# lucadellalib/audiocodecs

Measured on AMD Instinct MI355X. Metric: encode+decode audio-sec/s, EnCodec-24k 8cb, higher is better.
Workload: dtype f32 (GEMM-shaped kernels and LSTM products: operands as two scaled fp16 planes, 3 partial products, fp32 accumulate -- split16.h)

## Files before the change

audiocodecs_amd/csrc/ac_api.hip:

```cpp
#include "core.h"
#include "tap_route.h"

extern "C" {

int ac_version(void) { return 400; }

int ac_create(const ac_config* cfg, ac_handle** out) {
    if (!cfg || !out) return AC_EINVAL;
    *out = nullptr;
    if (cfg->struct_size != (int32_t)sizeof(ac_config)) return AC_EINVAL;
    if (cfg->num_ratios < 1 || cfg->num_ratios > AC_MAX_RATIOS || cfg->num_filters < 1 || cfg->hidden_size < 16 ||
        cfg->hidden_size % 16 || cfg->compress < 1 || cfg->num_lstm_layers < 1 || cfg->num_lstm_layers > 2 || cfg->codebook_size % 32 ||
        cfg->codebook_size < 16 || cfg->num_quantizers < 1 || cfg->kernel_size < 1 || cfg->kernel_size > 8 ||
        cfg->last_kernel_size < 1 || cfg->last_kernel_size > 8 || cfg->residual_kernel_size < 1 || cfg->residual_kernel_size > 8)
        return AC_EINVAL;
    int ndev = 0;
    if (hipGetDeviceCount(&ndev) != hipSuccess || ndev <= cfg->device || cfg->device < 0) return AC_ENODEV;
    ac_handle* h = new (std::nothrow) ac_handle();
    if (!h) return AC_ENOMEM;
    h->cfg = *cfg;
    h->hop = 1;
    for (int i = 0; i < cfg->num_ratios; ++i) h->hop *= cfg->upsampling_ratios[i];
    h->D = cfg->num_filters << cfg->num_ratios;
    *out = h;
// ... 16 lines not shown
    if (ends(".weight_g")) k = k.substr(0, k.size() - 9) + ".parametrizations.weight.original0";
    else if (ends(".weight_v")) k = k.substr(0, k.size() - 9) + ".parametrizations.weight.original1";
    return k;
}

int ac_load_weights(ac_handle* h, const char* name, const void* host_ptr, size_t bytes) {
    if (!h || !name || !host_ptr) return h ? fail(h, AC_EINVAL, "null argument") : AC_EINVAL;
    if (h->finalized) return fail(h, AC_ESTATE, "handle already finalized");
    if (bytes % 4) return fail(h, AC_EINVAL, "tensor '%s': byte size %zu is not a multiple of 4", name, bytes);
    const float* f = static_cast<const float*>(host_ptr);
    h->host[h->arch == ARCH_WAVTOK ? wavtok_key(name) : std::string(name)].assign(f, f + bytes / 4);
    return AC_OK;
}



static void latch_dev_switches(ac_handle* h) {
    auto num = [](const char* name, int dflt) { const char* v = std::getenv(name); return v && *v ? std::atoi(v) : dflt; };
    const char* e = std::getenv("AC_TAP_EPI");
    h->dev.tap_epi_staged = e && std::strcmp(e, "staged") == 0;
    h->dev.tap_dil = num("AC_TAP_DIL", 1);
    h->dev.tap_stagger = num("AC_TAP_STAGGER", 0);
    h->dev.tap_pick = num("AC_TAP_PICK", -1);
    h->dev.tap8 = num("AC_TAP8", -1);
    h->dev.tap8_form = num("AC_TAP8_FORM", 0);
    h->dev.tap8_spread = num("AC_TAP8_SPREAD", 1);
#ifdef AC_DEVELOPER
    h->dev.rb6_dbg = num("AC_RB6_DBG", 0);
    h->dev.lstm_dbg = num("AC_LSTM_DBG", 0);
#endif
    h->dev.rb_stream = num("AC_RB_STREAM", 1);
    h->dev.chain_stream = num("AC_CHAIN_STREAM", 1);
    h->dev.rb128_stream = num("AC_RB128_STREAM", 1);
    h->dev.front_seg = std::max(0, num("AC_FRONT_SEG", 0));
    h->dev.tail_seg = std::max(0, num("AC_TAIL_SEG", 0));
    h->dev.front_ldspad = std::max(0, num("AC_FRONT_LDSPAD", 0));
    h->dev.lstm_fuse_in = num("AC_LSTM_FUSE_IN", 1);
    const char* r = std::getenv("AC_RVQ");
    h->dev.rvq_exact = r && std::strcmp(r, "fp32") == 0;
    h->dev.prof_detail = num("AC_PROF_DETAIL", 0);
    h->dev.head_seq = num("AC_HEAD_SEQ", 0);
    h->dev.attn_exact = num("AC_ATTN_EXACT", 0);
    h->dev.dac_unit = num("AC_DAC_UNIT", 1);
    h->dev.mimi_tail = num("AC_MIMI_TAIL", 1);
    h->dev.mstream_skinny = num("AC_MSTREAM_SKINNY", -1);
}

int ac_debug_set(ac_handle* h, const char* key, int value) {
    if (!h || !key) return AC_EINVAL;
    struct { const char* k; int* v; } tab[] = {
        {"tap_epi_staged", &h->dev.tap_epi_staged}, {"tap_dil", &h->dev.tap_dil}, {"tap_stagger", &h->dev.tap_stagger}, {"tap_pick", &h->dev.tap_pick}, {"tap8", &h->dev.tap8}, {"tap8_form", &h->dev.tap8_form}, {"tap8_spread", &h->dev.tap8_spread},
        {"rb6_dbg", &h->dev.rb6_dbg}, {"rb_stream", &h->dev.rb_stream}, {"chain_stream", &h->dev.chain_stream}, {"rb128_stream", &h->dev.rb128_stream}, {"front_seg", &h->dev.front_seg}, {"tail_seg", &h->dev.tail_seg}, {"front_ldspad", &h->dev.front_ldspad},
        {"lstm_dbg", &h->dev.lstm_dbg}, {"lstm_fuse_in", &h->dev.lstm_fuse_in}, {"rvq_exact", &h->dev.rvq_exact}, {"prof_detail", &h->dev.prof_detail}, {"head_seq", &h->dev.head_seq}, {"attn_exact", &h->dev.attn_exact}, {"dac_unit", &h->dev.dac_unit}, {"mimi_tail", &h->dev.mimi_tail},
        {"mstream_skinny", &h->dev.mstream_skinny},
    };
#ifndef AC_DEVELOPER
    if (std::strcmp(key, "rb6_dbg") == 0 || std::strcmp(key, "lstm_dbg") == 0)
        return fail(h, AC_EINVAL, "ac_debug_set('%s'): a developer-build switch (timing modes with wrong results / fault injection); this is the product library", key);
#endif
    if (!h->finalized) return fail(h, AC_ESTATE, "ac_debug_set('%s'): the switches are latched by ac_finalize; set them afterwards", key);
    for (auto& t : tab)
        if (std::strcmp(t.k, key) == 0) {
            const bool nonneg = t.v == &h->dev.front_seg || t.v == &h->dev.tail_seg || t.v == &h->dev.front_ldspad || t.v == &h->dev.tap_stagger;
            if (nonneg && value < 0) return fail(h, AC_EINVAL, "ac_debug_set('%s', %d): the value must be >= 0", key, value);
            if (t.v == &h->dev.front_ldspad && value > 16384) return fail(h, AC_EINVAL, "ac_debug_set('front_ldspad', %d): at most 16384 bytes", value);
            if (t.v == &h->dev.tap8_form && (value < 0 || value > 5)) return fail(h, AC_EINVAL, "ac_debug_set('tap8_form', %d): 0 (cost model) .. 5", value);
            *t.v = value;
            return AC_OK;
        }
    return fail(h, AC_EINVAL, "ac_debug_set: unknown switch '%s'", key);
}

int ac_set_precision(ac_handle* h, int precision) {
    if (!h) return AC_EINVAL;
    if (h->finalized) return fail(h, AC_ESTATE, "ac_set_precision must precede ac_finalize (weights are packed for one arithmetic)");
    if (precision != AC_PRECISION_FP32 && precision != AC_PRECISION_FP32_EXACT) return fail(h, AC_EINVAL, "unknown precision %d", precision);
    h->precision = precision;
    return AC_OK;
}

int ac_finalize(ac_handle* h) {
    if (!h) return AC_EINVAL;
    if (h->finalized) return fail(h, AC_ESTATE, "handle already finalized");
    {
        int pr = h->precision;
// ... 587 lines not shown
```

audiocodecs_amd/csrc/core.h:

```cpp
#pragma once
#include <hip/hip_runtime.h>

#include <algorithm>
#include <cmath>
#include <cstdarg>
#include <cstdio>
#include <cstdlib>
#include <cstring>
#include <map>
#include <string>
#include <vector>

#include "../../include/audiocodecs_amd.h"
#include "lstm_consts.h"
#include "rvq_types.h"
#include "split16.h"
#include "tap_gemm.h"

using namespace ac;

namespace ac {
constexpr int THIN_MAXK = 8;
struct RbFused6Params;
}

namespace acimpl {


struct ConvSpec {
    std::string prefix;
    int transposed, cin, cout, k, s;
};

struct PackedGemm {
    size_t w_off = 0, b_off = 0;
    int N = 0, Ktot = 0;
    bool has_bias = true;
};

struct ResBlockPlan {
    int C;
    PackedGemm c3;
    PackedGemm fused;
    size_t w3f_off = 0, wff_off = 0;
    size_t winv3_off = 0, winvf_off = 0;
    size_t w3p_off = 0, wfp_off = 0;
    float hb0 = 0.f, hb1 = 0.f;
    bool has6 = false;
};

struct LstmPlan {
    int D, layers;
    std::vector<PackedGemm> ih;
    std::vector<size_t> hh_off;
    std::vector<size_t> ihpk_off;
    size_t persist_off = 0;
    size_t persist16_off = 0;
    size_t persist16_inv = 0;
    bool has_persist = false;
};

struct MimiTfLayer {
    PackedGemm qkv, o, fc1, fc2;
    size_t ln1_w = 0, ln1_b = 0, ln2_w = 0, ln2_b = 0, sc_a = 0, sc_m = 0;
};

struct MimiPlan {
    PackedGemm enc_stem, enc_final, down, dec_first, dec_head;
    std::vector<ResBlockPlan> enc_rb, dec_rb;
    std::vector<PackedGemm> enc_down, dec_up;
    std::vector<MimiTfLayer> enc_tf, dec_tf;
    size_t up_w = 0;
    PackedGemm in_proj;
    PackedGemm out_proj;
    size_t cb_plain = 0, cb_packed = 0, cb_ee = 0;
    size_t cb16 = 0, cb16_inv = 0;
    size_t rope_cos = 0, rope_sin = 0;
    int rope_T = 0;
    int D = 0;
    struct StreamM { size_t stem_f = 0, stem_inv = 0, head_f = 0, head_inv = 0; float sb0 = 0.f, sb1 = 0.f, fb0 = 0.f, fb1h = 0.f; bool stem_ok = false, head_ok = false; } sm;
};
// ... 58 lines not shown
    ac_mimi_config mcfg{};
    MimiPlan mimi;
    ac_dac_config dcfg{};
    DacPlan dac;
    ac_wavtok_config wcfg{};
    WavtokPlan wt;
    std::string err;
    std::map<std::string, std::vector<float>> host;
    bool finalized = false;
    float* blob = nullptr;
    size_t blob_floats = 0;
    int hop = 1, D = 0;
    PackedGemm enc_stem, enc_final;
    std::vector<ResBlockPlan> enc_rb;
    std::vector<PackedGemm> enc_down;
    LstmPlan enc_lstm, dec_lstm;
    PackedGemm dec_first, dec_head;
    std::vector<PackedGemm> dec_up;
    std::vector<ResBlockPlan> dec_rb;
    size_t cb_plain = 0, cb_packed = 0, cb_ee = 0;
    size_t cb16 = 0, cb16_inv = 0;
    struct ChainBounds { float sb0 = 0.f, sb1 = 0.f, fb0 = 0.f, fb1h = 0.f, fb1x = 0.f; bool ok = false; } enc_front, dec_tail;
    struct StreamImgs { size_t stem_f = 0, stem_inv = 0, down_f = 0, down_inv = 0, up_f = 0, up_inv = 0, head_f = 0, head_inv = 0; bool enc_ok = false, dec_ok = false; } simg;
    struct DevSwitches {
        int tap_epi_staged = 0;
        int tap_dil = 1;
        int tap_stagger = 0;
        int tap_pick = -1;
        int tap8 = -1;
        int tap8_form = 0;
        int tap8_spread = 1;
        int rb6_dbg = 0;
        int rb_stream = 1;
        int rb128_stream = 1;
        int chain_stream = 1;
        int front_seg = 0, tail_seg = 0;
        int front_ldspad = 0;
        int lstm_dbg = 0;
        int lstm_fuse_in = 1;
        int rvq_exact = 0;
        int prof_detail = 0;
        int attn_exact = 0;
        int dac_unit = 1;
        int mimi_tail = 1;
        int head_seq = 0;
        int mstream_skinny = -1;
    } dev;
    bool fuse_chains = true;
    float* dbg = nullptr;
    size_t dbg_cap = 0, dbg_used = 0;
    std::vector<const void*> lds_opted;
    std::map<size_t, size_t> w6_of;
    std::map<size_t, size_t> t6_of;
    std::map<size_t, size_t> t6inv_of;
    bool noncausal = false;
    bool has_enc = true, has_dec = true;
    bool gemm_fp32 = false;
    std::map<size_t, size_t> winv_of;
    std::map<const void*, int> mimi_streams;
    std::map<const void*, int> mimi_dstreams;
    struct EStreamReg {
        int B;
        std::vector<uint8_t> fresh;
    };
    std::map<const void*, EStreamReg> encodec_streams, encodec_dstreams;
    unsigned* amax_buf = nullptr;
// ... 207 lines not shown
        const int KS = H / 32;
        *img_off = reserve((size_t)Q * C * H);
        *inv_off = reserve((size_t)Q);
        std::vector<uint16_t> img((size_t)Q * C * H * 2);
        for (int q = 0; q < Q; ++q) {
            const float* e = &blob[plain + (size_t)q * C * H];
            const int se = row_scale(e, (size_t)C * H);
            blob[*inv_off + q] = s16_pow2(-se);
            for (int ct = 0; ct < C / 16; ++ct)
                for (int s = 0; s < KS; ++s)
                    for (int lane = 0; lane < 64; ++lane)
                        for (int e8 = 0; e8 < 8; ++e8) {
                            const int j = lane & 15, kq = lane >> 4;
                            const int dim = 16 * (2 * s + e8 / 4) + 4 * kq + e8 % 4;
                            uint16_t t[3];
                            split16h(e[(size_t)(ct * 16 + j) * H + dim], se, t);
                            const size_t base = ((((size_t)q * (C / 16) + ct) * KS + s) * 2) * 512 + (size_t)lane * 8 + e8;
                            img[base] = t[0];
                            img[base + 512] = t[1];
                        }
        }
        std::memcpy(&blob[*img_off], img.data(), img.size() * 2);
    }
    void pack_t6(const PackedGemm& g) {
        if (g.N != 64 || g.Ktot != 128 || !g.has_bias || h->t6_of.count(g.w_off)) return;
        std::vector<int> km(128);
        for (int k = 0; k < 128; ++k) km[k] = k;
        size_t ioff = 0;
        h->t6_of[g.w_off] = frag16(g.w_off, 64, 128, km, &ioff);
        if (use16()) h->t6inv_of[g.w_off] = ioff;
    }
    void rb6(ResBlockPlan& rb, bool sc) {
        const int C = rb.C, hid = C / 2;
        if ((C != 32 && C != 64 && C != 128) || rb.c3.N != hid || rb.c3.Ktot != 3 * C || rb.fused.N != C || rb.fused.Ktot != hid + (sc ? C : 0)) return;
        std::vector<int> k3(3 * C), kf;
        for (int k = 0; k < 3 * C; ++k) k3[k] = k;
        const int hcp = hid < 32 ? 32 : hid;
        for (int k = 0; k < hcp; ++k) kf.push_back(k < hid ? k : -1);
        for (int k = 0; sc && k < C; ++k) kf.push_back(hid + k);
        rb.w3f_off = frag16(rb.c3.w_off, hid, rb.c3.Ktot, k3, &rb.winv3_off);
        rb.wff_off = frag16(rb.fused.w_off, C, rb.fused.Ktot, kf, &rb.winvf_off);
        if ((C == 64 || C == 32 || C == 128) && use16()) {
            std::vector<int> k3p(k3.size()), kfp(kf.size());
            for (size_t k = 0; k < k3.size(); ++k) k3p[k] = k3[(k & ~(size_t)31) + ((k & 4) ? 16 : 0) + 4 * ((k >> 3) & 3) + (k & 3)];
            for (size_t k = 0; k < kf.size(); ++k) kfp[k] = kf[(k & ~(size_t)31) + ((k & 4) ? 16 : 0) + 4 * ((k >> 3) & 3) + (k & 3)];
            rb.w3p_off = frag16(rb.c3.w_off, hid, rb.c3.Ktot, k3p);
            rb.wfp_off = frag16(rb.fused.w_off, C, rb.fused.Ktot, kfp);
        }
        rb.hb0 = rb.hb1 = 0.f;
        for (int n = 0; n < hid; ++n) {
            double l1 = 0.0;
            for (int k = 0; k < rb.c3.Ktot; ++k) l1 += std::fabs((double)blob[rb.c3.w_off + (size_t)n * rb.c3.Ktot + k]);
            rb.hb1 = std::max(rb.hb1, (float)(l1 * 1.000001));
            rb.hb0 = std::max(rb.hb0, std::fabs(blob[rb.c3.b_off + n]));
        }
        rb.has6 = true;
    }
    bool conv(const ConvSpec& s, PackedGemm& g, bool bias = true) {
        std::vector<float> w;
        if (!weight(s, w)) return false;
        const std::vector<float>* b = bias ? get(s.prefix + ".bias", s.cout) : nullptr;
        if (bias && !b) return false;
        g.has_bias = bias;
        g.N = s.cout;
        g.Ktot = s.k * s.cin;
        g.w_off = reserve((size_t)g.N * g.Ktot);
// ... 306 lines not shown
const unsigned* amax_of(ac_handle* h, hipStream_t st, const float* x, long long bs, long long ts, int L, int C, int B, const unsigned* known);

unsigned* rowmax_new(ac_handle* h, hipStream_t st, long long rows, bool zero);

const unsigned* amax_plus(ac_handle* h, hipStream_t st, const Act& x, float add, int B);

TapSeg make_seg(const Act& x, int s, int J, int pad , int extra, int kofs, const float* rel_len, int left = -1, int right = 0);


inline bool aligned16(const void* p) { return (reinterpret_cast<uintptr_t>(p) & 15) == 0; }

int run_tap(ac_handle* h, hipStream_t st, TapGemmParams& p);


struct Out {
    float* raw = nullptr;
    float* elu = nullptr;
};

struct Act2 {
    Act raw{}, elu{};
};

int try_thin6(ac_handle* h, hipStream_t st, const PackedGemm& g, const Act& x, int width, int edge, Out out, int B, const unsigned** amax_out = nullptr);

int conv_fwd(ac_handle* h, hipStream_t st, const PackedGemm& g, const Act& x, int k, int s, const float* rel_len, Out out,
             long long out_bs, long long out_rs, int B, Act2* y);

int convtr_fwd(ac_handle* h, hipStream_t st, const PackedGemm& g, const Act& x, int s, Out out, int B, Act2* y);

bool rb128_ok(const ac_handle* h, const ResBlockPlan& rb);

int resblock_fwd(ac_handle* h, hipStream_t st, const ResBlockPlan& rb, const Act2& x, float* hbuf, Out out, int B, Act2* y);

bool thin_ok(const ac_config& c, int k);

int thin_stem(ac_handle* h, hipStream_t st, const PackedGemm& g, int F, int k, int pad, const float* sig, const float* rel_len, int B, int T,
              Out out, Act2* y, int padl = -1, const float* alpha = nullptr, const float* alpha_inv = nullptr, int Lp = -1);

int stem_fwd(ac_handle* h, hipStream_t st, const float* sig, const float* rel_len, int B, int T, Out out, Act2* y);

int thin_head(ac_handle* h, hipStream_t st, const PackedGemm& g, int F, int k, int pad, const Act& x, int B, float* sig, int padl = -1,
              int tanh_out = 0);

int head_fwd(ac_handle* h, hipStream_t st, const Act& x, int B, float* sig);

bool enc_front_ok(const ac_handle* h, int T);

int enc_front_fwd(ac_handle* h, hipStream_t st, const float* sig, const float* rel_len, int B, int T, float* y, float* dbg_x0, float* dbg_y1, Act2* out);

bool dec_tail_ok(const ac_handle* h, const Act& xe);

int dec_tail_fwd(ac_handle* h, hipStream_t st, const Act& xe, int B, float* sig, float* dbg_u, float* dbg_v);

void capture(ac_handle* h, hipStream_t st, const Act& a, int B);


struct LstmWs {
    float *gin, *gin1, *hseq0, *hseq1, *c;
};

int lstm_fwd(ac_handle* h, hipStream_t st, const LstmPlan& lp, const Act& x, const LstmWs& ws, Out out, int B, Act2* y);

int rvq_encode_fwd(ac_handle* h, hipStream_t st, const float* feats, int F, int K, long long* toks);

int rvq_decode_fwd(ac_handle* h, hipStream_t st, const long long* toks, int F, int K, float* out);
// ... 107 lines not shown
```

audiocodecs_amd/csrc/core.hip:

```cpp
#include "core.h"
#include "split16_kernels.h"
#include "lstm.h"
#include "lstm_persist.h"
#include "lstm_persist16.h"
#include "rvq.h"
#include "rvq16.h"
#include "tap_gemm4.h"
#include "tap_gemm6.h"
#include "tap_gemm8.h"
#include "tap_route.h"
#include "thin.h"
#include "rb_fused.h"
#include "rb_fused6.h"
#include "thin_conv6.h"
#include "rb_fused6_128.h"
#include "enc_front.h"
#include "dec_tail.h"

namespace acimpl {


int fail(ac_handle* h, int code, const char* fmt, ...) {
    char buf[1024];
    va_list ap;
    va_start(ap, fmt);
    vsnprintf(buf, sizeof buf, fmt, ap);
    va_end(ap);
    if (h) h->err = buf;
    return code;
}


int ensure_lds(ac_handle* h, const void* func, size_t bytes) {
    if (bytes <= 64 * 1024) return AC_OK;
    for (const void* f : h->lds_opted)
        if (f == func) return AC_OK;
    HIPCHK(h, hipFuncSetAttribute(func, hipFuncAttributeMaxDynamicSharedMemorySize, (int)bytes));
    h->lds_opted.push_back(func);
    return AC_OK;
}


Arch make_arch(const ac_config& c) {
    Arch a;
    const int F = c.num_filters, H = c.hidden_size, n = c.num_ratios;
    auto P = [](const char* part, int i, const char* rest) {
        return std::string(part) + ".layers." + std::to_string(i) + rest;
    };
// ... 526 lines not shown
    using Cfg = Rb128Cfg<SC>;
    RbFused6Params p{};
    p.xr = x.raw.p;
    p.w3f = reinterpret_cast<const __bf16*>(h->blob + rb.w3f_off);
    p.wff = reinterpret_cast<const __bf16*>(h->blob + rb.wff_off);
    p.b3 = h->blob + rb.c3.b_off;
    p.bf = h->blob + rb.fused.b_off;
    p.y = out.raw;
    p.y_elu = out.elu;
    p.B = B;
    p.L = x.raw.L;
    p.lpad = h->noncausal ? 1 : 2;
    p.Lp = x.raw.L > p.lpad ? x.raw.L : p.lpad + 1;
    p.ntiles = cdiv(x.raw.L, Cfg::BM);
    p.pad = pad;
    if (!rb_split16(h, st, rb, x, B, p, amax_out)) return fail(h, AC_ESTATE, "fused residual block without split16 images");
    if (!p.amax_in) return fail(h, AC_ESTATE, "out of amax slots (split16.h)");
    if (h->dev.rb_stream && h->dev.rb128_stream && p.lpad == 2 && pad == (SC ? PAD_REFLECT : PAD_ZERO) && rb.w3p_off && (long long)x.raw.L * 512 < 0x70000000LL)
        return launch_rb_stream128m(h, st, p, rb, SC, out, B);
    if (int rc = ensure_lds(h, reinterpret_cast<const void*>(rb128_fused6_kernel<SC, 2>), Cfg::lds_bytes)) return rc;
    const long long total = (long long)B * p.ntiles;
    const int grid = (int)std::min<long long>(total, 256);
    const double L = x.raw.L;
    ProfScope ps(h, st, SC ? "rb128_fused6_kernel<true, 2>" : "rb128_fused6_kernel<false, 2>",
                 2.0 * B * L * (64.0 * 384 + 128.0 * (64 + (SC ? 128 : 0))),
                 (double)B * L * 128 * 4.0 * (1 + (out.raw ? 1 : 0) + (out.elu ? 1 : 0)));
    hipLaunchKernelGGL((rb128_fused6_kernel<SC, 2>), dim3(grid), dim3(512), Cfg::lds_bytes, st, p);
    return AC_OK;
}

bool rb128_ok(const ac_handle* h, const ResBlockPlan& rb) { return rb.C == 128 && rb.has6 && !h->gemm_fp32; }


int resblock_fwd(ac_handle* h, hipStream_t st, const ResBlockPlan& rb, const Act2& x, float* hbuf, Out out, int B, Act2* y) {
    if (rb128_ok(h, rb) && h->cfg.residual_kernel_size == 3 && h->cfg.compress == 2 && x.raw.ts == 128 &&
        x.raw.bs == (long long)x.raw.L * 128 && aligned16(x.raw.p) && (long long)x.raw.L * 512 < 0x70000000LL) {
        const unsigned* am = nullptr;
        int rc = launch_rb128_fused6<true>(h, st, rb, x, out, B, PAD_REFLECT, &am);
        if (rc) return rc;
        HIPCHK(h, hipGetLastError());
        const long long bs = (long long)x.raw.L * 128;
        y->raw = Act{out.raw, bs, 128, x.raw.L, 128, am, B};
        y->elu = Act{out.elu, bs, 128, x.raw.L, 128, am, B};
        return AC_OK;
    }
    if ((rb.C == 32 || rb.C == 64) && !(h->noncausal && (!rb.has6 || h->gemm_fp32)) && h->cfg.residual_kernel_size == 3 && h->cfg.compress == 2 && x.raw.ts == rb.C &&
        x.raw.bs == (long long)x.raw.L * rb.C && aligned16(x.raw.p) &&
        (!x.elu.p || (x.elu.ts == rb.C && x.elu.bs == x.raw.bs && aligned16(x.elu.p)))) {
        int rc;
        const unsigned* am = nullptr;
        if (rb.has6 && !h->gemm_fp32) rc = rb.C == 32 ? launch_rb_fused6<32, true>(h, st, rb, x, out, B, PAD_REFLECT, &am) : launch_rb_fused6<64, true>(h, st, rb, x, out, B, PAD_REFLECT, &am);
        else rc = rb.C == 32 ? launch_rb_fused<32, 128, 1>(h, st, rb, x, out, B) : launch_rb_fused<64, 64, 2>(h, st, rb, x, out, B);
        if (rc) return rc;
        HIPCHK(h, hipGetLastError());
        const long long bs = (long long)x.raw.L * rb.C;
        y->raw = Act{out.raw, bs, rb.C, x.raw.L, rb.C, am, B};
        y->elu = Act{out.elu, bs, rb.C, x.raw.L, rb.C, am, B};
        return AC_OK;
    }
    Act2 hv;
    int rc = conv_fwd(h, st, rb.c3, x.elu, h->cfg.residual_kernel_size, 1, nullptr, Out{nullptr, hbuf},
                      (long long)x.elu.L * rb.c3.N, rb.c3.N, B, &hv);
    if (rc) return rc;
    TapGemmParams p{};
    p.nseg = 2;
    p.seg[0] = make_seg(hv.elu, 1, 1, PAD_REFLECT, 0, 0, nullptr);
    p.seg[1] = make_seg(x.raw, 1, 1, PAD_REFLECT, 0, hv.elu.C, nullptr);
    p.w = h->blob + rb.fused.w_off;
    p.bias = h->blob + rb.fused.b_off;
    p.y = out.raw;
    p.y_elu = out.elu;
    p.y_bs = (long long)x.raw.L * rb.C;
    p.y_rs = rb.C;
    p.B = B;
    p.M = x.raw.L;
    p.N = rb.C;
    p.Ktot = rb.fused.Ktot;
    rc = run_tap(h, st, p);
    y->raw = Act{out.raw, p.y_bs, p.y_rs, x.raw.L, rb.C, p.amax_out, p.B};
    y->elu = Act{out.elu, p.y_bs, p.y_rs, x.raw.L, rb.C, p.amax_out, p.B};
    return rc;
}


bool thin_ok(const ac_config& c, int k) { return c.num_filters % 4 == 0 && c.num_filters <= 64 && k <= THIN_MAXK; }


int thin_stem(ac_handle* h, hipStream_t st, const PackedGemm& g, int F, int k, int pad, const float* sig, const float* rel_len, int B, int T,
              Out out, Act2* y, int padl, const float* alpha, const float* alpha_inv, int Lp) {
    ThinParams p{};
    p.padl = padl < 0 ? k - 1 : padl;
    p.alpha = alpha;
// ... 530 lines not shown
            char lstm[400] = "", tok[200] = "";
            if (a || b) {
                h->lstm_step_only = true;
                std::snprintf(lstm, sizeof lstm,
                              "an EARLIER call's persistent LSTM launch failed (%u bounded waits expired, %u launches without 32 workgroups on "
                              "every XCD -- is the GPU shared?): that call's outputs were set to NaN; the handle now uses the per-step LSTM "
                              "kernels, repeat the call", a, b);
            }
            if (t) std::snprintf(tok, sizeof tok, "an EARLIER ac_decode / ac_dequantize call got %u token ids outside [0, codebook_size): those frames were set to NaN", t);
            return fail(h, (a || b) ? AC_EHIP : AC_EINVAL, "%s%s%s", lstm, (a || b) && t ? "; ALSO: " : "", tok);
        }
    }
    return AC_OK;
}


int check_len(ac_handle* h, long long samples) {
    const long long lim = 0x70000000LL / (h->arch == ARCH_DAC ? 512 : 256) - 1;
    if (samples > lim) return fail(h, AC_EINVAL, "clip of %lld samples is too long for one call (limit %lld): split it", samples, lim);
    return AC_OK;
}


int encoder_fwd(ac_handle* h, hipStream_t st, const float* sig, const float* rel_len, int B, int T, float* feats, WsPtrs& ws) {
    const ac_config& c = h->cfg;
    const bool dbg = h->dbg != nullptr;
    Act xin{sig, (long long)T, 1, T, 1};
    Act2 x, y;
    int rc;
    auto rb_self_elu = [&](int C) {
        if (h->noncausal && h->gemm_fp32) return false;
        return (C == 32 || C == 64 || (C == 128 && c.num_ratios > 2 && rb128_ok(h, h->enc_rb[2]))) && c.residual_kernel_size == 3 && c.compress == 2;
    };
    int i0 = 0;
    if (enc_front_ok(h, T)) {
        float* d0 = dbg ? ws.take() : nullptr;
        float* d1 = dbg ? ws.take() : nullptr;
        rc = enc_front_fwd(h, st, sig, rel_len, B, T, ws.take(), d0, d1, &x);
        if (rc) return rc;
        if (dbg) {
            capture(h, st, Act{d0, (long long)T * 32, 32, T, 32}, B);
            capture(h, st, Act{d1, (long long)T * 32, 32, T, 32}, B);
            ws.give(d0);
            ws.give(d1);
        }
        capture(h, st, x.raw, B);
        i0 = 1;
    } else {
    if (thin_ok(c, c.kernel_size))
        rc = stem_fwd(h, st, sig, rel_len, B, T, Out{ws.take(), rb_self_elu(c.num_filters) ? nullptr : ws.take()}, &x);
    else
        rc = conv_fwd(h, st, h->enc_stem, xin, c.kernel_size, 1, rel_len, Out{ws.take(), ws.take()},
                      (long long)T * c.num_filters, c.num_filters, B, &x);
    if (rc) return rc;
    capture(h, st, x.raw, B);
    }
    for (int i = i0; i < c.num_ratios; ++i) {
        const int ratio = c.upsampling_ratios[c.num_ratios - 1 - i];
        float* hb = ws.take();
        rc = resblock_fwd(h, st, h->enc_rb[i], x, hb, Out{dbg ? ws.take() : nullptr, ws.take()}, B, &y);
        if (rc) return rc;
        ws.give(hb);
        ws.give(x);
        if (dbg) { capture(h, st, y.raw, B); ws.give(y.raw.p); y.raw.p = nullptr; }
        x = y;
        const int M = cdiv(x.elu.L, ratio);
        const bool last = i == c.num_ratios - 1;
        rc = conv_fwd(h, st, h->enc_down[i], x.elu, 2 * ratio, ratio, nullptr,
                      Out{ws.take(), (last || rb_self_elu(h->enc_down[i].N)) ? nullptr : ws.take()},
                      (long long)M * h->enc_down[i].N, h->enc_down[i].N, B, &y);
        if (rc) return rc;
        ws.give(x);
        x = y;
        capture(h, st, x.raw, B);
    }
    rc = lstm_fwd(h, st, h->enc_lstm, x.raw, ws.lstm, Out{dbg ? ws.take() : nullptr, ws.take()}, B, &y);
    if (rc) return rc;
    ws.give(x);
    if (dbg) { capture(h, st, y.raw, B); ws.give(y.raw.p); y.raw.p = nullptr; }
    x = y;
    rc = conv_fwd(h, st, h->enc_final, x.elu, c.last_kernel_size, 1, nullptr, Out{feats, nullptr},
                  (long long)x.elu.L * c.hidden_size, c.hidden_size, B, nullptr);
    ws.give(x);
    return rc;
}


int decoder_fwd(ac_handle* h, hipStream_t st, const long long* toks, int B, int N, int K, float* sig, WsPtrs& ws) {
    const ac_config& c = h->cfg;
    const bool dbg = h->dbg != nullptr;
    float* zb = ws.take();
    int rc = rvq_decode_fwd(h, st, toks, B * N, K, zb);
    if (rc) return rc;
    Act z{zb, (long long)N * c.hidden_size, c.hidden_size, N, c.hidden_size};
    Act2 x, y;
    rc = conv_fwd(h, st, h->dec_first, z, c.kernel_size, 1, nullptr, Out{ws.take(), nullptr}, (long long)N * h->D, h->D, B, &x);
    if (rc) return rc;
    ws.give(zb);
    capture(h, st, x.raw, B);
    rc = lstm_fwd(h, st, h->dec_lstm, x.raw, ws.lstm, Out{dbg ? ws.take() : nullptr, ws.take()}, B, &y);
    if (rc) return rc;
    ws.give(x);
    if (dbg) { capture(h, st, y.raw, B); ws.give(y.raw.p); y.raw.p = nullptr; }
    x = y;
    for (int i = 0; i < c.num_ratios; ++i) {
        if (i == c.num_ratios - 1 && dec_tail_ok(h, x.elu)) {
            const long long T2 = 2LL * x.elu.L;
            float* d0 = dbg ? ws.take() : nullptr;
            float* d1 = dbg ? ws.take() : nullptr;
            rc = dec_tail_fwd(h, st, x.elu, B, sig, d0, d1);
            if (rc) return rc;
            if (dbg) {
                capture(h, st, Act{d0, T2 * 32, 32, (int)T2, 32}, B);
                capture(h, st, Act{d1, T2 * 32, 32, (int)T2, 32}, B);
                ws.give(d0);
                ws.give(d1);
            }
            ws.give(x);
            return AC_OK;
        }
        const int cup = h->dec_up[i].N / c.upsampling_ratios[i];
        const bool self_elu = (cup == 32 || cup == 64 || (cup == 128 && rb128_ok(h, h->dec_rb[i]))) && c.residual_kernel_size == 3 &&
                              c.compress == 2;
        rc = convtr_fwd(h, st, h->dec_up[i], x.elu, c.upsampling_ratios[i], Out{ws.take(), self_elu ? nullptr : ws.take()}, B, &y);
        if (rc) return rc;
        ws.give(x);
        x = y;
        capture(h, st, x.raw, B);
        float* hb = ws.take();
        rc = resblock_fwd(h, st, h->dec_rb[i], x, hb, Out{dbg ? ws.take() : nullptr, ws.take()}, B, &y);
        if (rc) return rc;
        ws.give(hb);
        ws.give(x);
        if (dbg) { capture(h, st, y.raw, B); ws.give(y.raw.p); y.raw.p = nullptr; }
        x = y;
    }
    if (thin_ok(c, c.last_kernel_size) && x.elu.ts == c.num_filters)
        rc = head_fwd(h, st, x.elu, B, sig);
    else
        rc = conv_fwd(h, st, h->dec_head, x.elu, c.last_kernel_size, 1, nullptr, Out{sig, nullptr}, (long long)x.elu.L, 1, B, nullptr);
    ws.give(x);
    return rc;
}

int mimi_linear(ac_handle* h, hipStream_t st, const PackedGemm& g, const float* x, long long rows, int cin, int x_pitch, int kofs,
                float* y, int y_pitch, const Epi& epi) {
    const long long widest = std::max<long long>(std::max(x_pitch, y_pitch), g.N);
    long long chunk = ((1LL << 31) / 4 - 4096) / widest / 128 * 128;
    if (chunk < 128) return fail(h, AC_EINVAL, "linear layer too wide for the tap-GEMM (%lld)", widest);
    for (long long r0 = 0; r0 < rows; r0 += chunk) {
        const long long n = std::min(chunk, rows - r0);
        TapGemmParams p{};
        p.nseg = 1;
        Act xa{x + r0 * x_pitch, 0, x_pitch, (int)n, cin};
        const bool one = r0 == 0 && n == rows;
        if (one && epi.rowmax_in) { xa.amax = epi.rowmax_in; xa.amax_n = -(int)n; }
// ... 134 lines not shown
```

audiocodecs_amd/csrc/tap_gemm6.h:

```cpp
#pragma once
#include "tap_gemm4.h"
#include "split16.h"
#include <type_traits>

namespace ac {

typedef __bf16 bf16x8 __attribute__((ext_vector_type(8)));
typedef float f32x16 __attribute__((ext_vector_type(16)));

__device__ __forceinline__ void lds_barrier() {
    asm volatile("s_waitcnt lgkmcnt(0)" ::: "memory");
    __builtin_amdgcn_s_barrier();
    asm volatile("" ::: "memory");
}

constexpr int T6_PITCH = 40;

template <int WGM, int WGN, int WMT, int WN, int HALO = 7>
struct Tap6Cfg {
    static_assert((WGM * WGN == 4 || WGM * WGN == 8) && (WGM * WMT == 4 || WGM * WMT == 8), "4 or 8 waves, 128 or 256 rows");
    static constexpr int BM = 32 * WGM * WMT, BN = 32 * WGN * WN, NT = 64 * WGM * WGN;
    static constexpr int A_ROWS = BM + HALO;
    static constexpr int A_SLOTS = (A_ROWS * (KC / 4) + NT - 1) / NT;
    static constexpr int PLANE = A_ROWS * T6_PITCH;
// ... 232 lines not shown
                        w.x = snake1(v.x, al.x, ai.x); w.y = snake1(v.y, al.y, ai.y); w.z = snake1(v.z, al.z, ai.z); w.w = snake1(v.w, al.w, ai.w);
                        if (p.amax_out) amax_acc4(omax, w);
                    } else {
                        w = elu4(v);
                    }
                    *reinterpret_cast<f32x4*>(p.y_elu + o) = w;
                }
            }
            if (NP == 2 && p.amax_out_rows) {
                rmax = group_max_u32<CW / 4>(rmax);
                if (q == 0 && m < p.M && rmax) atomicMax(p.amax_out_rows + m, rmax);
            }
        }
#ifdef T6_TRACE
        if (c == 0 && a0 == 0) T6_PHASE(10);
#endif
    }
#ifdef T6_TRACE
    T6_PHASE(11);
#endif
    if (p.amax_out) amax_flush(omax, amax_at(p.amax_out, b));
#ifdef T6_TRACE
    T6_PHASE(9);
#endif
    if (p.clk && tid == 0) {
        atomicAdd(&p.clk[0], (unsigned long long)(__builtin_amdgcn_s_memtime() - clk_t0));
        atomicAdd(&p.clk[1], (unsigned long long)(__builtin_amdgcn_s_memrealtime() - clk_r0));
    }
}

struct Tap6Tile {
    int b, m0, n0;
    float a_inv;
    bool rowmode;
    unsigned long long clk_t0, clk_r0;
    bool t6_ph;
};

template <int WGM, int WGN, int WMT, int WN, int HALO, bool SWAP>
__device__ __forceinline__ void tap6_mainloop(const TapGemmParams& p, const __bf16* __restrict__ wp, float* smem, f32x16 (&acc)[WMT][WN], Tap6Tile& tl) {
    constexpr int NP = 2;
    using Cfg = Tap6Cfg<WGM, WGN, WMT, WN, HALO>;
    constexpr int BM = Cfg::BM, BN = Cfg::BN, NT = Cfg::NT, A_SLOTS = Cfg::A_SLOTS, PLANE = Cfg::PLANE;
    unsigned long long clk_t0 = 0, clk_r0 = 0;
    if (p.clk) { clk_t0 = __builtin_amdgcn_s_memtime(); clk_r0 = __builtin_amdgcn_s_memrealtime(); }
    if (p.stagger && (int)blockIdx.x < 256 * tap6_occupancy<WGM, WGN, WMT, WN, NP>()) {
        const unsigned long long wait = (unsigned long long)((blockIdx.x * 0x9E3779B1u) >> 24) * (unsigned)p.stagger >> 8;
        const unsigned long long t0 = __builtin_amdgcn_s_memtime();
        while (__builtin_amdgcn_s_memtime() - t0 < wait) __builtin_amdgcn_s_sleep(32);
    }
    __bf16* As0 = reinterpret_cast<__bf16*>(smem);
    constexpr int NPL = 2;

    const int tid = threadIdx.x, lane = tid & 63;
    const int wave = __builtin_amdgcn_readfirstlane(tid >> 6);
    const int wm = wave / WGN, wn = wave % WGN;
    const int i32 = lane & 31, kh = lane >> 5;

    int id;
    {
        const int total = gridDim.x, q = total >> 3, r = total & 7, xcd = blockIdx.x & 7, pos = blockIdx.x >> 3;
        id = (xcd < r ? xcd * (q + 1) : r * (q + 1) + (xcd - r) * q) + pos;
    }
    const int nt = id % p.ntiles; id /= p.ntiles;
    const int mt = id % p.mtiles;
    const int b = id / p.mtiles;
    const int m0 = mt * BM, n0 = nt * BN;
    const unsigned am_e0 = *amax_at(p.seg[0].amax, b);
    const unsigned am_e1 = *amax_at(p.seg[p.nseg > 1 ? 1 : 0].amax, b);
#ifdef T6_TRACE
    const bool t6_ph = p.clk && mt == p.mtiles / 2 && nt == 0 && b == p.B / 2 && tid == 64;
    if (t6_ph) p.clk[4] = clk_t0;
    T6_PHASE(1);
#endif

#pragma unroll
    for (int a = 0; a < WMT; ++a)
#pragma unroll
        for (int c = 0; c < WN; ++c)
#pragma unroll
            for (int r = 0; r < 16; ++r) acc[a][c][r] = 0.f;

    static_assert(NT % (KC / 4) == 0, "slots are whole rows apart");
    int a_boff[A_SLOTS];
    const int a_lds0 = (tid / (KC / 4)) * T6_PITCH + 4 * (tid % (KC / 4));
    const bool last_slot_ok = (tid + (A_SLOTS - 1) * NT) / (KC / 4) < Cfg::A_ROWS;

    int si = 0, c0 = 0, j = 0;
    int seg_J, seg_Cw, seg_kofs;
    int seg_tapoff = 0;
    bool seg_reload = false;
    int seg_rowstep = 1;
    bool seg_interior;
    unsigned a_zero = 0;
    __amdgpu_buffer_rsrc_t a_rs;
    auto enter_segment = [&](int s_) {
        const TapSeg& sg = p.seg[s_];
        seg_J = sg.J;
        seg_Cw = sg.s * sg.cin;
        seg_kofs = sg.kofs;
        seg_reload = sg.dil != 1 && (sg.s != 1 || (sg.J - 1) * sg.dil > HALO);
        seg_rowstep = seg_reload ? 1 : sg.dil;
        const long long lo = (long long)m0 * sg.s - sg.pad;
        const long long hi = (long long)(m0 + BM - 1 + (sg.J - 1) * sg.dil) * sg.s + (sg.s - 1) - sg.pad;
        const bool inside = lo >= 0 && hi < sg.L;
        seg_interior = inside || (sg.s == 1 && !seg_reload);
        a_zero = 0;
        const int tsf = sg.s == 1 ? (int)sg.ts : sg.cin;
        seg_tapoff = sg.dil * sg.s * tsf * 4;
        a_rs = __builtin_amdgcn_make_buffer_rsrc((void*)(sg.x + (long long)b * sg.bs), 0,
                                                 (int)(((long long)(sg.L - 1) * sg.ts + sg.cin) * 4), 0x00020000);
        const int R = seg_reload ? BM : BM + (sg.J - 1) * sg.dil;
#pragma unroll
        for (int i = 0; i < A_SLOTS; ++i) {
            const int e = tid + i * NT;
            const int row = e / (KC / 4), q = e % (KC / 4);
            long long t = (long long)(m0 + (row < R ? row : 0)) * sg.s - sg.pad;
            if (!inside) {
                if (sg.s == 1 && !seg_reload) {
                    const long long jj = row < R ? src_index(sg, (int)t) : 0;
                    if (jj < 0) a_zero |= 1u << i;
                    t = jj < 0 ? 0 : jj;
                } else {
                    t = 0;
                }
            }
            a_boff[i] = (int)((t * tsf + 4 * q) * 4);
        }
    };
    constexpr bool CAN_ROWMODE = HALO == 7;
    constexpr int NRSC = CAN_ROWMODE ? A_SLOTS : 1;
    float a_scale = 1.f, a_inv = 1.f;
    float a_rsc[NRSC];
    const bool rowmode = CAN_ROWMODE && NP == 2 && p.amax_rows;
    unsigned am_rows[NRSC];
#pragma unroll
    for (int i = 0; i < NRSC; ++i) {
        const int m = m0 + (tid + i * NT) / (KC / 4);
        am_rows[i] = p.seg[0].amax[rowmode ? (m < p.M ? m : p.M - 1) : 0];
    }
    auto set_scales = [&]() {
        if (!rowmode) {
            unsigned a0 = am_e0, a1 = am_e1;
            asm volatile("" : "+v"(a0), "+v"(a1));
            const int se = s16_exponent(a1 > a0 ? a1 : a0);
            a_scale = s16_pow2(se);
            a_inv = s16_pow2(-se);
        }
#pragma unroll
        for (int i = 0; i < NRSC; ++i) a_rsc[i] = rowmode ? s16_pow2(s16_exponent(am_rows[i])) : a_scale;
    };
    f32x4 ra[A_SLOTS];
    constexpr int A_OOB = 0x7fff0000;
    auto load_a = [&](int s_, int c_, int j_, bool live) {
#ifdef T6_ABL_NOALOAD
        live = false;
#endif
        int voff[A_SLOTS], soff = 0;
        if (seg_interior || !live) {
            soff = __builtin_amdgcn_readfirstlane(live ? c_ * 4 + (seg_reload ? j_ * seg_tapoff : 0) : 0);
#pragma unroll
            for (int i = 0; i < A_SLOTS; ++i) voff[i] = live ? a_boff[i] : A_OOB;
        } else {
            const TapSeg& sg = p.seg[s_];
            const int R = seg_reload ? BM : BM + (sg.J - 1) * sg.dil;
            const int jr = seg_reload ? j_ * sg.dil : 0;
#pragma unroll
            for (int i = 0; i < A_SLOTS; ++i) {
                const int e = tid + i * NT;
                const int row = e / (KC / 4), q = e % (KC / 4);
                const int c = c_ + 4 * q;
                const int tp = sg.cin_shift >= 0 ? (c >> sg.cin_shift) : (c / sg.cin);
                const long long jj = row < R ? src_index(sg, (m0 + row + jr) * sg.s + tp - sg.pad) : -1;
                voff[i] = jj < 0 ? A_OOB : (int)((jj * sg.ts + (c - tp * sg.cin)) * 4);
            }
        }
#pragma unroll
        for (int i = 0; i < A_SLOTS; ++i) ra[i] = bufload16(a_rs, voff[i], soff);
    };
    auto store_a = [&](__bf16* dst) {
#ifdef T6_ABL_NOSTORE
#pragma unroll
        for (int i = 0; i < A_SLOTS; ++i) asm volatile("" ::"v"(ra[i]));
        return;
#endif
#pragma unroll
        for (int i = 0; i < A_SLOTS; ++i)
            if (i + 1 < A_SLOTS || last_slot_ok) {
                const f32x4 v = (a_zero & (1u << i)) ? f32x4{0.f, 0.f, 0.f, 0.f} : ra[i];
                split16_store4s(v, a_rsc[CAN_ROWMODE ? i : 0], dst, PLANE, a_lds0 + i * (NT / (KC / 4)) * T6_PITCH);
            }
    };
    const int ksteps = p.Ktot >> 4;
    constexpr int WPL = 2;
    const __bf16* wbase = wp + ((long long)((n0 + wn * 32 * WN) >> 5) * ksteps) * (WPL * 64 * 8) + lane * 8;
    auto load_b = [&](int s_, bf16x8 (&bf)[3][WN]) {
#ifdef T6_ABL_NOBLOAD
        asm volatile("" : "+v"(bf[0][0]), "+v"(bf[1][0]));
        return;
#endif
#pragma unroll
        for (int c = 0; c < WN; ++c)
#pragma unroll
            for (int pl = 0; pl < NP; ++pl)
                bf[pl][c] = *reinterpret_cast<const bf16x8*>(wbase + (((long long)c * ksteps + s_) * WPL + pl) * (64 * 8));
    };

#ifdef T6_TRACE
    T6_PHASE(2);
#endif
    enter_segment(0);
#ifdef T6_TRACE
    T6_PHASE(3);
#endif
    load_a(0, 0, 0, true);
    bf16x8 bx[3][WN], by[3][WN], bz[3][WN];
    load_b(seg_kofs >> 4, bx);
    load_b((seg_kofs >> 4) + 1, by);
#ifdef T6_TRACE
    T6_PHASE(4);
#endif
    __builtin_amdgcn_sched_barrier(0);
// ... 152 lines not shown
```

Measured before the change: 41820.

## Fuse C=256 residual block into one kernel with on-chip hidden activations

Adds a fused residual-block kernel for 256-channel blocks. It computes the k=3 conv with ELU applied while staging its input, keeps the 128-channel hidden activation as split fp16 planes in LDS, and accumulates the 1x1 conv plus the skip GEMM into the same accumulators. This removes the intermediate hidden buffer round trip, a launch, and the separate ELU'd copy of the block input, since upstream convs now skip writing it. The cost is heavier LDS and register use per workgroup and a custom scaling bound derived from weight L1 norms.

Result: faster. 42270 (median of 6 runs) (+1.1%).

```diff
diff --git a/audiocodecs_amd/csrc/ac_api.hip b/audiocodecs_amd/csrc/ac_api.hip
--- a/audiocodecs_amd/csrc/ac_api.hip
+++ b/audiocodecs_amd/csrc/ac_api.hip
@@ -72,6 +72,7 @@
     h->dev.rb_stream = num("AC_RB_STREAM", 1);
     h->dev.chain_stream = num("AC_CHAIN_STREAM", 1);
     h->dev.rb128_stream = num("AC_RB128_STREAM", 1);
+    h->dev.rb256_fused = num("AC_RB256_FUSED", 1);
     h->dev.front_seg = std::max(0, num("AC_FRONT_SEG", 0));
     h->dev.tail_seg = std::max(0, num("AC_TAIL_SEG", 0));
     h->dev.front_ldspad = std::max(0, num("AC_FRONT_LDSPAD", 0));
@@ -90,7 +91,7 @@
     if (!h || !key) return AC_EINVAL;
     struct { const char* k; int* v; } tab[] = {
         {"tap_epi_staged", &h->dev.tap_epi_staged}, {"tap_dil", &h->dev.tap_dil}, {"tap_stagger", &h->dev.tap_stagger}, {"tap_pick", &h->dev.tap_pick}, {"tap8", &h->dev.tap8}, {"tap8_form", &h->dev.tap8_form}, {"tap8_spread", &h->dev.tap8_spread},
-        {"rb6_dbg", &h->dev.rb6_dbg}, {"rb_stream", &h->dev.rb_stream}, {"chain_stream", &h->dev.chain_stream}, {"rb128_stream", &h->dev.rb128_stream}, {"front_seg", &h->dev.front_seg}, {"tail_seg", &h->dev.tail_seg}, {"front_ldspad", &h->dev.front_ldspad},
+        {"rb6_dbg", &h->dev.rb6_dbg}, {"rb_stream", &h->dev.rb_stream}, {"chain_stream", &h->dev.chain_stream}, {"rb128_stream", &h->dev.rb128_stream}, {"rb256_fused", &h->dev.rb256_fused}, {"front_seg", &h->dev.front_seg}, {"tail_seg", &h->dev.tail_seg}, {"front_ldspad", &h->dev.front_ldspad},
         {"lstm_dbg", &h->dev.lstm_dbg}, {"lstm_fuse_in", &h->dev.lstm_fuse_in}, {"rvq_exact", &h->dev.rvq_exact}, {"prof_detail", &h->dev.prof_detail}, {"head_seq", &h->dev.head_seq}, {"attn_exact", &h->dev.attn_exact}, {"dac_unit", &h->dev.dac_unit}, {"mimi_tail", &h->dev.mimi_tail},
         {"mstream_skinny", &h->dev.mstream_skinny},
     };
diff --git a/audiocodecs_amd/csrc/core.h b/audiocodecs_amd/csrc/core.h
--- a/audiocodecs_amd/csrc/core.h
+++ b/audiocodecs_amd/csrc/core.h
@@ -47,6 +47,7 @@
     size_t w3p_off = 0, wfp_off = 0;
     float hb0 = 0.f, hb1 = 0.f;
     bool has6 = false;
+    bool hb256 = false;
 };
 
 struct LstmPlan {
@@ -171,6 +172,7 @@
         int tap8_spread = 1;
         int rb6_dbg = 0;
         int rb_stream = 1;
+        int rb256_fused = 1;
         int rb128_stream = 1;
         int chain_stream = 1;
         int front_seg = 0, tail_seg = 0;
@@ -444,6 +446,17 @@
     }
     void rb6(ResBlockPlan& rb, bool sc) {
         const int C = rb.C, hid = C / 2;
+        if (C == 256 && sc && use16() && rb.c3.N == hid && rb.c3.Ktot == 3 * C && rb.fused.N == C && rb.fused.Ktot == hid + C && rb.c3.has_bias && rb.fused.has_bias) {
+            rb.hb0 = rb.hb1 = 0.f;
+            for (int n = 0; n < hid; ++n) {
+                double l1 = 0.0;
+                for (int k = 0; k < rb.c3.Ktot; ++k) l1 += std::fabs((double)blob[rb.c3.w_off + (size_t)n * rb.c3.Ktot + k]);
+                rb.hb1 = std::max(rb.hb1, (float)(l1 * 1.000001));
+                rb.hb0 = std::max(rb.hb0, std::fabs(blob[rb.c3.b_off + n]));
+            }
+            rb.hb256 = true;
+            return;
+        }
         if ((C != 32 && C != 64 && C != 128) || rb.c3.N != hid || rb.c3.Ktot != 3 * C || rb.fused.N != C || rb.fused.Ktot != hid + (sc ? C : 0)) return;
         std::vector<int> k3(3 * C), kf;
         for (int k = 0; k < 3 * C; ++k) k3[k] = k;
@@ -816,6 +829,7 @@
 bool rb128_ok(const ac_handle* h, const ResBlockPlan& rb);
 
 int resblock_fwd(ac_handle* h, hipStream_t st, const ResBlockPlan& rb, const Act2& x, float* hbuf, Out out, int B, Act2* y);
+bool rb256_ok(const ac_handle* h, const ResBlockPlan& rb, int L);
 
 bool thin_ok(const ac_config& c, int k);
 
diff --git a/audiocodecs_amd/csrc/core.hip b/audiocodecs_amd/csrc/core.hip
--- a/audiocodecs_amd/csrc/core.hip
+++ b/audiocodecs_amd/csrc/core.hip
@@ -14,6 +14,7 @@
 #include "rb_fused6.h"
 #include "thin_conv6.h"
 #include "rb_fused6_128.h"
+#include "rb256_fused.h"
 #include "enc_front.h"
 #include "dec_tail.h"
 
@@ -606,6 +607,68 @@
 bool rb128_ok(const ac_handle* h, const ResBlockPlan& rb) { return rb.C == 128 && rb.has6 && !h->gemm_fp32; }
 
 
+bool rb256_ok(const ac_handle* h, const ResBlockPlan& rb, int L) {
+    if (!h->dev.rb256_fused || rb.C != 256 || !rb.hb256 || h->gemm_fp32 || h->noncausal || h->cfg.residual_kernel_size != 3 || h->cfg.compress != 2 || L < Rb256Cfg::BM ||
+        (long long)L * 1024 >= 0x70000000LL)
+        return false;
+    return h->w6_of.count(rb.c3.w_off) && h->winv_of.count(rb.c3.w_off) && h->w6_of.count(rb.fused.w_off) && h->winv_of.count(rb.fused.w_off);
+}
+
+int launch_rb256_fused(ac_handle* h, hipStream_t st, const ResBlockPlan& rb, const Act2& x, Out out, int B, Act2* y) {
+    using Cfg = Rb256Cfg;
+    const int L = x.raw.L;
+    const unsigned* am = amax_of(h, st, x.raw.p, x.raw.bs, x.raw.ts, L, 256, B, x.raw.amax_n == B ? x.raw.amax : nullptr);
+    if (!am) return fail(h, AC_ESTATE, "out of amax slots (split16.h)");
+    Act xr = x.raw;
+    xr.amax = am;
+    xr.amax_n = B;
+    Rb256Params q{};
+    TapGemmParams& a = q.a;
+    a.nseg = 1;
+    a.seg[0] = make_seg(xr, 1, 3, PAD_REFLECT, 0, 0, nullptr);
+    a.w = h->blob + rb.c3.w_off;
+    a.bias = h->blob + rb.c3.b_off;
+    a.winv = h->blob + h->winv_of.at(rb.c3.w_off);
+    a.B = B;
+    a.M = L;
+    a.N = rb.c3.N;
+    a.Ktot = rb.c3.Ktot;
+    a.mtiles = cdiv(L, Cfg::BM);
+    a.ntiles = 1;
+    TapGemmParams& b = q.b;
+    b.nseg = 1;
+    b.seg[0] = make_seg(xr, 1, 1, PAD_REFLECT, 0, rb.c3.N, nullptr);
+    b.w = h->blob + rb.fused.w_off;
+    b.bias = h->blob + rb.fused.b_off;
+    b.winv = h->blob + h->winv_of.at(rb.fused.w_off);
+    b.y = out.raw;
+    b.y_elu = out.elu;
+    b.y_bs = (long long)L * 256;
+    b.y_rs = 256;
+    b.B = B;
+    b.M = L;
+    b.N = 256;
+    b.Ktot = rb.fused.Ktot;
+    b.mtiles = a.mtiles;
+    b.ntiles = 1;
+    b.amax_out = amax_new(h);
+    b.epi_direct = h->dev.tap_epi_staged ? 0 : 1;
+    q.hb0 = rb.hb0;
+    q.hb1 = rb.hb1;
+    if (int rc = ensure_lds(h, reinterpret_cast<const void*>(rb256_fused_kernel), Cfg::lds_bytes)) return rc;
+    {
+        ProfScope ps(h, st, "rb256_fused_kernel", 2.0 * B * (double)L * (128.0 * 768 + 256.0 * 384),
+                     (double)B * L * 256 * 4.0 * (1 + (out.raw ? 1 : 0) + (out.elu ? 1 : 0)) + (128.0 * 768 + 256.0 * 384) * 4.0);
+        hipLaunchKernelGGL(rb256_fused_kernel, dim3((unsigned)((long long)B * a.mtiles)), dim3(Cfg::NT), Cfg::lds_bytes, st, q,
+                           reinterpret_cast<const __bf16*>(h->blob + h->w6_of.at(rb.c3.w_off)), reinterpret_cast<const __bf16*>(h->blob + h->w6_of.at(rb.fused.w_off)));
+    }
+    HIPCHK(h, hipGetLastError());
+    y->raw = Act{out.raw, b.y_bs, 256, L, 256, b.amax_out, B};
+    y->elu = Act{out.elu, b.y_bs, 256, L, 256, b.amax_out, B};
+    return AC_OK;
+}
+
+
 int resblock_fwd(ac_handle* h, hipStream_t st, const ResBlockPlan& rb, const Act2& x, float* hbuf, Out out, int B, Act2* y) {
     if (rb128_ok(h, rb) && h->cfg.residual_kernel_size == 3 && h->cfg.compress == 2 && x.raw.ts == 128 &&
         x.raw.bs == (long long)x.raw.L * 128 && aligned16(x.raw.p) && (long long)x.raw.L * 512 < 0x70000000LL) {
@@ -618,6 +681,9 @@
         y->elu = Act{out.elu, bs, 128, x.raw.L, 128, am, B};
         return AC_OK;
     }
+    if (rb256_ok(h, rb, x.raw.L) && x.raw.ts == 256 && x.raw.bs == (long long)x.raw.L * 256 && aligned16(x.raw.p) && (out.raw == nullptr || aligned16(out.raw)) &&
+        aligned16(out.elu))
+        return launch_rb256_fused(h, st, rb, x, out, B, y);
     if ((rb.C == 32 || rb.C == 64) && !(h->noncausal && (!rb.has6 || h->gemm_fp32)) && h->cfg.residual_kernel_size == 3 && h->cfg.compress == 2 && x.raw.ts == rb.C &&
         x.raw.bs == (long long)x.raw.L * rb.C && aligned16(x.raw.p) &&
         (!x.elu.p || (x.elu.ts == rb.C && x.elu.bs == x.raw.bs && aligned16(x.elu.p)))) {
@@ -632,6 +698,7 @@
         y->elu = Act{out.elu, bs, rb.C, x.raw.L, rb.C, am, B};
         return AC_OK;
     }
+    if (!x.elu.p) return fail(h, AC_ESTATE, "residual block: the two-launch path needs the ELU'd flavour of its input");
     Act2 hv;
     int rc = conv_fwd(h, st, rb.c3, x.elu, h->cfg.residual_kernel_size, 1, nullptr, Out{nullptr, hbuf},
                       (long long)x.elu.L * rb.c3.N, rb.c3.N, B, &hv);
@@ -1228,6 +1295,7 @@
         if (h->noncausal && h->gemm_fp32) return false;
         return (C == 32 || C == 64 || (C == 128 && c.num_ratios > 2 && rb128_ok(h, h->enc_rb[2]))) && c.residual_kernel_size == 3 && c.compress == 2;
     };
+    auto rb256_self_elu = [&](int i, int L) { return i < c.num_ratios && h->enc_rb[i].C == h->enc_down[i - 1].N && rb256_ok(h, h->enc_rb[i], L); };
     int i0 = 0;
     if (enc_front_ok(h, T)) {
         float* d0 = dbg ? ws.take() : nullptr;
@@ -1263,7 +1331,7 @@
         const int M = cdiv(x.elu.L, ratio);
         const bool last = i == c.num_ratios - 1;
         rc = conv_fwd(h, st, h->enc_down[i], x.elu, 2 * ratio, ratio, nullptr,
-                      Out{ws.take(), (last || rb_self_elu(h->enc_down[i].N)) ? nullptr : ws.take()},
+                      Out{ws.take(), (last || rb_self_elu(h->enc_down[i].N) || rb256_self_elu(i + 1, M)) ? nullptr : ws.take()},
                       (long long)M * h->enc_down[i].N, h->enc_down[i].N, B, &y);
         if (rc) return rc;
         ws.give(x);
@@ -1316,8 +1384,9 @@
             return AC_OK;
         }
         const int cup = h->dec_up[i].N / c.upsampling_ratios[i];
-        const bool self_elu = (cup == 32 || cup == 64 || (cup == 128 && rb128_ok(h, h->dec_rb[i]))) && c.residual_kernel_size == 3 &&
-                              c.compress == 2;
+        const bool self_elu = ((cup == 32 || cup == 64 || (cup == 128 && rb128_ok(h, h->dec_rb[i]))) && c.residual_kernel_size == 3 &&
+                               c.compress == 2) ||
+                              (cup == h->dec_rb[i].C && rb256_ok(h, h->dec_rb[i], x.elu.L * c.upsampling_ratios[i]));
         rc = convtr_fwd(h, st, h->dec_up[i], x.elu, c.upsampling_ratios[i], Out{ws.take(), self_elu ? nullptr : ws.take()}, B, &y);
         if (rc) return rc;
         ws.give(x);
diff --git a/audiocodecs_amd/csrc/rb256_fused.h b/audiocodecs_amd/csrc/rb256_fused.h
--- /dev/null
+++ b/audiocodecs_amd/csrc/rb256_fused.h
@@ -0,0 +1,107 @@
+#pragma once
+#include "tap_gemm6.h"
+#include "rb_params6.h"
+
+namespace ac {
+
+struct Rb256Params {
+    TapGemmParams a;
+    TapGemmParams b;
+    float hb0, hb1;
+};
+
+struct Rb256Cfg {
+    using CA = Tap6Cfg<1, 4, 4, 1, 7>;
+    using CB = Tap6Cfg<1, 4, 4, 2, 7>;
+    static constexpr int BM = 128, HC = 128, NT = 256;
+    static constexpr int HP = HC + 8;
+    static constexpr int H_PLANE = BM * HP;
+    static constexpr size_t h_bytes = (size_t)2 * H_PLANE * 2;
+    static constexpr size_t ab_bytes = CA::lds_bytes > CB::lds_bytes ? CA::lds_bytes : CB::lds_bytes;
+    static constexpr size_t lds_bytes = h_bytes > ab_bytes ? h_bytes : ab_bytes;
+    static_assert(CA::BM == BM && CB::BM == BM && CA::BN == HC && CB::BN == 256 && 2 * lds_bytes <= 160 * 1024, "one tile shape; two workgroups per CU");
+};
+
+__global__ __launch_bounds__(256, 2) void rb256_fused_kernel(const Rb256Params q, const __bf16* __restrict__ wa, const __bf16* __restrict__ wb) {
+    using Cfg = Rb256Cfg;
+    constexpr int HP = Cfg::HP, H_PLANE = Cfg::H_PLANE;
+    extern __shared__ __attribute__((aligned(16))) float smem[];
+    const int tid = threadIdx.x, lane = tid & 63;
+    const int wn = __builtin_amdgcn_readfirstlane(tid >> 6);
+    const int i32 = lane & 31, kh = lane >> 5;
+    _Float16* Hs = reinterpret_cast<_Float16*>(smem);
+    Tap6Tile tl;
+    f32x16 acc[4][2];
+    {
+        f32x16 acc_a[4][1];
+        tap6_mainloop<1, 4, 4, 1, 7, false, 1>(q.a, wa, smem, acc_a, tl);
+        const Rb16Scale cs = rb16_scale(*amax_at(q.a.seg[0].amax, tl.b), q.hb0, q.hb1);
+        const int ng = wn * 32 + i32;
+        const float bv = q.a.bias[ng];
+        const float iv = tl.a_inv * q.a.winv[ng];
+        lds_barrier();
+#pragma unroll
+        for (int a = 0; a < 4; ++a)
+#pragma unroll
+            for (int r = 0; r < 16; ++r) {
+                const int row = a * 32 + 8 * (r / 4) + 4 * kh + (r % 4);
+                const float v = elu1(__fmaf_rn(acc_a[a][0][r], iv, bv));
+                const _Float16 hi = (_Float16)(v * cs.sb);
+                const _Float16 lo = (_Float16)__builtin_fmaf(v, cs.sb, -(float)hi);
+                Hs[row * HP + ng] = hi;
+                Hs[H_PLANE + row * HP + ng] = lo;
+            }
+        tl.a_scale = cs.sb;
+        tl.a_inv = cs.ib;
+    }
+    lds_barrier();
+
+#pragma unroll
+    for (int a = 0; a < 4; ++a)
+#pragma unroll
+        for (int c = 0; c < 2; ++c)
+#pragma unroll
+            for (int r = 0; r < 16; ++r) acc[a][c][r] = 0.f;
+    {
+        const int ksteps = q.b.Ktot >> 4;
+        const __bf16* wbase = wb + ((long long)(wn * 2) * ksteps) * (2 * 64 * 8) + lane * 8;
+        auto load_b = [&](int s, bf16x8 (&bf)[2][2]) {
+#pragma unroll
+            for (int c = 0; c < 2; ++c)
+#pragma unroll
+                for (int pl = 0; pl < 2; ++pl) bf[pl][c] = *reinterpret_cast<const bf16x8*>(wbase + (((long long)c * ksteps + s) * 2 + pl) * (64 * 8));
+        };
+        const _Float16* Ha = Hs + i32 * HP + 8 * kh;
+        auto step = [&](int s, const bf16x8 (&bf)[2][2]) {
+            f16x8 af[2][4];
+#pragma unroll
+            for (int pl = 0; pl < 2; ++pl)
+#pragma unroll
+                for (int a = 0; a < 4; ++a) af[pl][a] = *reinterpret_cast<const f16x8*>(Ha + pl * H_PLANE + a * 32 * HP + s * 16);
+#pragma unroll
+            for (int a = 0; a < 4; ++a)
+#pragma unroll
+                for (int c = 0; c < 2; ++c) {
+                    f32x16 v = acc[a][c];
+                    v = __builtin_amdgcn_mfma_f32_32x32x16_f16(af[1][a], __builtin_bit_cast(f16x8, bf[0][c]), v, 0, 0, 0);
+                    v = __builtin_amdgcn_mfma_f32_32x32x16_f16(af[0][a], __builtin_bit_cast(f16x8, bf[1][c]), v, 0, 0, 0);
+                    acc[a][c] = __builtin_amdgcn_mfma_f32_32x32x16_f16(af[0][a], __builtin_bit_cast(f16x8, bf[0][c]), v, 0, 0, 0);
+                }
+        };
+        bf16x8 b0[2][2], b1[2][2];
+        load_b(0, b0);
+#pragma unroll
+        for (int s = 0; s < Cfg::HC / 16; s += 2) {
+            load_b(s + 1, b1);
+            step(s, b0);
+            if (s + 2 < Cfg::HC / 16) load_b(s + 2, b0);
+            step(s + 1, b1);
+        }
+    }
+    lds_barrier();
+
+    tap6_mainloop<1, 4, 4, 2, 7, false, 2>(q.b, wb, smem, acc, tl);
+    tap6_epilogue<1, 4, 4, 2, 7>(q.b, acc, smem, tl.b, tl.m0, tl.n0, tl.a_inv, false, tl.clk_t0, tl.clk_r0, false);
+}
+
+}
diff --git a/audiocodecs_amd/csrc/tap_gemm6.h b/audiocodecs_amd/csrc/tap_gemm6.h
--- a/audiocodecs_amd/csrc/tap_gemm6.h
+++ b/audiocodecs_amd/csrc/tap_gemm6.h
@@ -288,19 +288,21 @@
 struct Tap6Tile {
     int b, m0, n0;
     float a_inv;
+    float a_scale;
     bool rowmode;
     unsigned long long clk_t0, clk_r0;
     bool t6_ph;
 };
 
-template <int WGM, int WGN, int WMT, int WN, int HALO, bool SWAP>
+template <int WGM, int WGN, int WMT, int WN, int HALO, bool SWAP, int FUSE = 0>
 __device__ __forceinline__ void tap6_mainloop(const TapGemmParams& p, const __bf16* __restrict__ wp, float* smem, f32x16 (&acc)[WMT][WN], Tap6Tile& tl) {
     constexpr int NP = 2;
     using Cfg = Tap6Cfg<WGM, WGN, WMT, WN, HALO>;
     constexpr int BM = Cfg::BM, BN = Cfg::BN, NT = Cfg::NT, A_SLOTS = Cfg::A_SLOTS, PLANE = Cfg::PLANE;
     unsigned long long clk_t0 = 0, clk_r0 = 0;
-    if (p.clk) { clk_t0 = __builtin_amdgcn_s_memtime(); clk_r0 = __builtin_amdgcn_s_memrealtime(); }
-    if (p.stagger && (int)blockIdx.x < 256 * tap6_occupancy<WGM, WGN, WMT, WN, NP>()) {
+    if (FUSE == 2) { clk_t0 = tl.clk_t0; clk_r0 = tl.clk_r0; }
+    else if (p.clk) { clk_t0 = __builtin_amdgcn_s_memtime(); clk_r0 = __builtin_amdgcn_s_memrealtime(); }
+    if (FUSE != 2 && p.stagger && (int)blockIdx.x < 256 * tap6_occupancy<WGM, WGN, WMT, WN, NP>()) {
         const unsigned long long wait = (unsigned long long)((blockIdx.x * 0x9E3779B1u) >> 24) * (unsigned)p.stagger >> 8;
         const unsigned long long t0 = __builtin_amdgcn_s_memtime();
         while (__builtin_amdgcn_s_memtime() - t0 < wait) __builtin_amdgcn_s_sleep(32);
@@ -330,12 +332,14 @@
     T6_PHASE(1);
 #endif
 
-#pragma unroll
-    for (int a = 0; a < WMT; ++a)
-#pragma unroll
-        for (int c = 0; c < WN; ++c)
-#pragma unroll
-            for (int r = 0; r < 16; ++r) acc[a][c][r] = 0.f;
+    if constexpr (FUSE != 2) {
+#pragma unroll
+        for (int a = 0; a < WMT; ++a)
+#pragma unroll
+            for (int c = 0; c < WN; ++c)
+#pragma unroll
+                for (int r = 0; r < 16; ++r) acc[a][c][r] = 0.f;
+    }
 
     static_assert(NT % (KC / 4) == 0, "slots are whole rows apart");
     int a_boff[A_SLOTS];
@@ -396,7 +400,10 @@
         am_rows[i] = p.seg[0].amax[rowmode ? (m < p.M ? m : p.M - 1) : 0];
     }
     auto set_scales = [&]() {
-        if (!rowmode) {
+        if constexpr (FUSE == 2) {
+            a_scale = tl.a_scale;
+            a_inv = tl.a_inv;
+        } else if (!rowmode) {
             unsigned a0 = am_e0, a1 = am_e1;
             asm volatile("" : "+v"(a0), "+v"(a1));
             const int se = s16_exponent(a1 > a0 ? a1 : a0);
@@ -443,7 +450,8 @@
 #pragma unroll
         for (int i = 0; i < A_SLOTS; ++i)
             if (i + 1 < A_SLOTS || last_slot_ok) {
-                const f32x4 v = (a_zero & (1u << i)) ? f32x4{0.f, 0.f, 0.f, 0.f} : ra[i];
+                f32x4 v = (a_zero & (1u << i)) ? f32x4{0.f, 0.f, 0.f, 0.f} : ra[i];
+                if constexpr (FUSE == 1) v = elu4(v);
                 split16_store4s(v, a_rsc[CAN_ROWMODE ? i : 0], dst, PLANE, a_lds0 + i * (NT / (KC / 4)) * T6_PITCH);
             }
     };
```
